# kscalelabs/kbot-joystick

Measured on AMD Instinct MI355X. Metric: env-steps/sec (whole node), K-Bot joystick 8192 envs @1/2/4/8 MI355X, higher is better.
Workload: dtype f32; 1 GPU; kbot-headless, 8192 envs/GPU, flat ground, fixed joystick command (0.5,0,0), full iteration: 100-step rollout + PPO update (batch 512/GPU, 3 passes, LSTM hidden 256, depth 2); envs_per_gpu=8192, rollout_steps=100, batch_size_per_gpu=512, num_passes=3, hidden_size=256, deterministic_update=True, parallelism=env-sharded dp1, grad all-reduce per optimizer step

## Files before the change

### kbot-joystick_amd/csrc/kbj_nn.hip

```cpp
#include <hip/hip_runtime.h>
#include <vector>
#include <cmath>
#include <cstdlib>
#include <algorithm>
#include <type_traits>
#include "kbj_ctx.h"
#include "kbj_gemm.h"
#include "kbj_nn_kernels.h"
#include "kbj_lstm_seq.h"
#include "kbj_lstm_bwd16.h"

using namespace kbj;

namespace {

constexpr int MAXD = KBJ_MAX_DEPTH;

struct NetOff {
  size_t w_in, b_in, w_ih[MAXD], w_hh[MAXD], b[MAXD], w_out, b_out;
  int nin, nout, ld_obs;
};

struct TrainBufs {
  float *obs, *X0, *G[MAXD], *Hm[MAXD], *Hout[MAXD], *Cm[MAXD], *TanhC[MAXD], *Out, *dOut, *dHa, *dHb, *dGl[MAXD];
// ... 122 lines not shown
  void* q = nullptr;
  hipError_t e = hipMalloc(&q, count * sizeof(T));
  if (e != hipSuccess) return kbj_fail(ctx, std::string("hipMalloc (nn workspace): ") + hipGetErrorString(e));
  w.allocs.push_back(q);
  *p = reinterpret_cast<T*>(q);
  return 0;
}

constexpr int g_fold_sk = 8;
#ifndef KBJ_SPLITK_WGS
#define KBJ_SPLITK_WGS 768
#endif
constexpr int g_splitk_wgs = KBJ_SPLITK_WGS;
constexpr int DETP_ROWS = 512, DETP_COLS = 4 * 512;

int lane_of(kbj_ctx* ctx, hipStream_t s) { return s == ctx->stream ? 0 : (s == ctx->stream2 ? 1 : (s == ctx->side[0] ? 2 : 3)); }
float* sk_workspace(kbj_ctx* ctx, hipStream_t s, size_t floats) {
  NnWs& w = *ws_of(ctx);
  if (!w.sched.deterministic) return nullptr;
  const int l = lane_of(ctx, s);
  if (w.skws_cap[l] < floats) {
    hipDeviceSynchronize();
    if (w.skws[l]) hipFree(w.skws[l]);
    w.skws[l] = nullptr; w.skws_cap[l] = 0;
    void* q = nullptr;
    if (hipMalloc(&q, floats * sizeof(float)) != hipSuccess) { kbj_fail(ctx, "hipMalloc (deterministic split-K workspace)"); return nullptr; }
    w.skws[l] = reinterpret_cast<float*>(q); w.skws_cap[l] = floats;
  }
  return w.skws[l];
}
float* det_partials(kbj_ctx* ctx, hipStream_t s) {
  NnWs& w = *ws_of(ctx);
  return w.sched.deterministic ? w.detp[lane_of(ctx, s)] : nullptr;
}

inline dim3 g1(size_t n, int bs = 256) { return dim3((unsigned)((n + bs - 1) / bs)); }

void linear_fwd(hipStream_t s, const float* x, int lda, const float* W, int ldw, const float* bias, float* y, int ldy, int M, int N, int K, int beta) {
  GemmArgs g{x, W, y, bias, M, N, K, lda, ldw, ldy, beta, 1, nullptr};
  gemm_launch<true, true>(s, g);
}
void linear_bwd_input(hipStream_t s, bool x3, const float* dy, int lddy, const float* W, int ldw, float* dx, int lddx, int M, int N, int K, int beta, int tile = -1) {
  GemmArgs g{dy, W, dx, nullptr, M, N, K, lddy, ldw, lddx, beta, 1, nullptr};
  g.x3 = x3;
  gemm_launch<true, false>(s, g, x3 ? -1 : tile);
}
void linear_bwd_weight(kbj_ctx* ctx, hipStream_t s, bool x3, const float* dy, int lddy, const float* x, int ldx, float* dW, int lddw, int Nout, int Nin, int R) {
  bool big = Nout >= 128 && Nin >= 128;
  int ts = big ? 128 : 64;
  int tiles = ((Nout + ts - 1) / ts) * ((Nin + ts - 1) / ts);
  int sk = std::max(2, std::min(256, g_splitk_wgs / std::max(1, tiles)));
  sk = std::max(2, std::min(sk, (R + 255) / 256));
  GemmArgs g{dy, x, dW, nullptr, Nout, Nin, R, lddy, ldx, lddw, 1, sk, nullptr};
  g.skws = sk_workspace(ctx, s, (size_t)sk * Nout * Nin);
  g.x3 = x3;
  gemm_launch<false, false>(s, g, big ? 1 : 0);
}

void linear_bwd_weight2(kbj_ctx* ctx, hipStream_t s, bool x3, const float* dy, int lddy, const float* x1, const float* x2, int ldx, float* dW1, float* dW2, int lddw, int Nout, int Nin, int R) {
  bool big = Nout >= 128 && Nin >= 128;
  int ts = big ? 128 : 64;
  if (Nin % ts != 0) {
    linear_bwd_weight(ctx, s, x3, dy, lddy, x1, ldx, dW1, lddw, Nout, Nin, R);
    linear_bwd_weight(ctx, s, x3, dy, lddy, x2, ldx, dW2, lddw, Nout, Nin, R);
    return;
  }
  int tiles = ((Nout + ts - 1) / ts) * (2 * Nin / ts);
  int sk = std::max(2, std::min(256, g_splitk_wgs / std::max(1, tiles)));
  sk = std::max(2, std::min(sk, (R + 255) / 256));
  GemmArgs g{dy, x1, dW1, nullptr, Nout, 2 * Nin, R, lddy, ldx, lddw, 1, sk, nullptr};
  g.B2 = x2; g.C2 = dW2; g.n1 = Nin;
  g.skws = sk_workspace(ctx, s, (size_t)sk * Nout * 2 * Nin);
  g.x3 = x3;
  gemm_launch<false, false>(s, g, big ? 1 : 0);
}
void colsum_acc(kbj_ctx* ctx, hipStream_t s, const float* X, int M, int N, int ld, float* out) {
  float* part = det_partials(ctx, s);
  hipLaunchKernelGGL(colsum_kernel, dim3((N + 63) / 64, DETP_ROWS), dim3(256), 0, s, X, M, N, ld, out, part);
  if (part) reduce_rows_launch(s, part, DETP_ROWS, N, out);
}

constexpr int SEQ_UW = 2;
constexpr int SEQ_FUSED_MAX_H = 256;
constexpr int SEQ_MAX_H = 512;
constexpr int SEQ_COUNTER_WORDS = 256;
constexpr int SEQ_COUNTER_TOTAL = 2 * MAXD * 4 * SEQ_COUNTER_WORDS;

template <int HC = 64, class F> bool dispatch_hidden(int H, F&& f) {
  if constexpr (HC > SEQ_MAX_H) return false;
  else return H == HC ? f(std::integral_constant<int, HC>()) : dispatch_hidden<HC + 64>(H, f);
}

int seq_fwd(kbj_ctx* ctx, hipStream_t st, int H, const SeqFwdArgs& a0) {
  SeqFwdArgs a = a0;
  a.timeout_ticks = ws_of(ctx)->seq_timeout_ticks;
  KbjKernelTimer timer(st, a.X ? (a.ldx == KBJ_LD_ACTOR ? KBJ_KIND_SEQ_FWD_OBS : KBJ_KIND_SEQ_FWD_FUSED) : KBJ_KIND_SEQ_FWD, 2.0 * a.T * a.B * 4.0 * H * (H + (a.X ? (a.kx ? a.kx : H) : 0)));
  const bool built = dispatch_hidden(H, [&](auto hc) {
    constexpr int HC = decltype(hc)::value, UW = SEQ_UW;
    int grid = (HC / (SEQ_UNITS * UW)) * ((a.B + SEQ_ROWS - 1) / SEQ_ROWS);
    if (ctx->set.seq_drop > 0 && grid > 1) { --ctx->set.seq_drop; --grid; }
    const dim3 block(256 * UW);
    if constexpr (HC <= SEQ_FUSED_MAX_H) {
      if (a.X && a.ldx == KBJ_LD_ACTOR) { hipLaunchKernelGGL((lstm_seq_fwd_kernel<HC, UW, true, KBJ_LD_ACTOR>), dim3(grid), block, 0, st, a); return true; }
      if (a.X) { hipLaunchKernelGGL((lstm_seq_fwd_kernel<HC, UW, true>), dim3(grid), block, 0, st, a); return true; }
    }
    hipLaunchKernelGGL((lstm_seq_fwd_kernel<HC, UW, false>), dim3(grid), block, 0, st, a);
    return true;
  });
  return built ? 0 : kbj_fail(ctx, "seq_fwd: the persistent LSTM kernels are built for hidden sizes 64, 128, ..., 512");
}
int seq_bwd_row_groups(int B, bool tiles16) { return tiles16 ? (B + BWD16_ROWS - 1) / BWD16_ROWS : (B + SEQ_ROWS - 1) / SEQ_ROWS; }
int seq_bwd(kbj_ctx* ctx, hipStream_t st, int H, const SeqBwdArgs& a0, bool tiles16 = false) {
  SeqBwdArgs a = a0;
  a.timeout_ticks = ws_of(ctx)->seq_timeout_ticks;
  KbjKernelTimer timer(st, tiles16 ? KBJ_KIND_SEQ_BWD16 : KBJ_KIND_SEQ_BWD, 2.0 * a.T * a.B * 4.0 * H * H);
  const bool built = dispatch_hidden(H, [&](auto hc) {
    constexpr int HC = decltype(hc)::value, UW = SEQ_UW;
    if (tiles16) {
      if constexpr (HC <= SEQ_FUSED_MAX_H) {
        int grid = (HC / BWD16_UNITS) * ((a.B + BWD16_ROWS - 1) / BWD16_ROWS);
        if (ctx->set.seq_drop_bwd > 0 && grid > 1 && HC > BWD16_UNITS) { --ctx->set.seq_drop_bwd; --grid; }
        hipLaunchKernelGGL((lstm_seq_bwd16_kernel<HC>), dim3(grid), dim3(BWD16_NTH), 0, st, a);
        return true;
      } else return false;
    }
    const dim3 grid((HC / (SEQ_UNITS * UW)) * ((a.B + SEQ_ROWS - 1) / SEQ_ROWS)), block(256 * UW);
    if constexpr (HC <= SEQ_FUSED_MAX_H) hipLaunchKernelGGL((lstm_seq_bwd_kernel<HC, UW>), grid, block, 0, st, a);
    else hipLaunchKernelGGL((lstm_seq_bwd_wide_kernel<HC, UW>), grid, block, 0, st, a);
    return true;
  });
  return built ? 0 : kbj_fail(ctx, "seq_bwd: the persistent LSTM kernels are built for hidden sizes 64, 128, ..., 512 (lstm_seq_bwd16_kernel: up to 256)");
}

template <int H> hipError_t seq_min_blocks_per_cu(int* out) {
  constexpr int threads = 256 * SEQ_UW;
  int n[4] = {0, 0, 0, 0};
  hipError_t e = hipOccupancyMaxActiveBlocksPerMultiprocessor(&n[2], lstm_seq_fwd_kernel<H, SEQ_UW, false, H>, threads, 0);
  if constexpr (H <= SEQ_FUSED_MAX_H) {
    if (e == hipSuccess) e = hipOccupancyMaxActiveBlocksPerMultiprocessor(&n[0], lstm_seq_fwd_kernel<H, SEQ_UW, true, H>, threads, 0);
    if (e == hipSuccess) e = hipOccupancyMaxActiveBlocksPerMultiprocessor(&n[1], lstm_seq_fwd_kernel<H, SEQ_UW, true, KBJ_LD_ACTOR>, threads, 0);
    if (e == hipSuccess) e = hipOccupancyMaxActiveBlocksPerMultiprocessor(&n[3], lstm_seq_bwd_kernel<H, SEQ_UW>, threads, 0);
    int n16 = 0;
    if (e == hipSuccess) e = hipOccupancyMaxActiveBlocksPerMultiprocessor(&n16, lstm_seq_bwd16_kernel<H>, BWD16_NTH, 0);
    n[3] = std::min(n[3], n16);
  } else {
    if (e == hipSuccess) e = hipOccupancyMaxActiveBlocksPerMultiprocessor(&n[3], lstm_seq_bwd_wide_kernel<H, SEQ_UW>, threads, 0);
    n[0] = n[1] = n[2];
  }
  *out = std::min(std::min(n[0], n[1]), std::min(n[2], n[3]));
  return e;
}

int lstm_step(kbj_ctx* ctx, hipStream_t st, int H, const StepArgs& a) {
  const bool obs = a.ldx == KBJ_LD_ACTOR && a.ldw == KBJ_LD_ACTOR;
  KbjKernelTimer timer(st, obs ? KBJ_KIND_LSTM_STEP_OBS : KBJ_KIND_LSTM_STEP, 2.0 * a.M * 4.0 * H * (H + (a.kx ? a.kx : H)));
  const int nug = H / (SEQ_UNITS * 2), nrg = (a.M + SEQ_ROWS - 1) / SEQ_ROWS;
  const int nch = std::max(1, std::min(nrg, 256 / nug));
  dim3 grid(nug * nch), block(512);
  const bool built = dispatch_hidden(H, [&](auto hc) {
    constexpr int HC = decltype(hc)::value;
    if constexpr (HC <= SEQ_FUSED_MAX_H) {
      if (obs) hipLaunchKernelGGL((lstm_step_kernel<HC, 2, KBJ_LD_ACTOR>), grid, block, 0, st, a);
      else hipLaunchKernelGGL((lstm_step_kernel<HC, 2>), grid, block, 0, st, a);
      return true;
    } else return false;
  });
  return built ? 0 : kbj_fail(ctx, "lstm_step: the LSTM step kernels are built for hidden_size 64, 128, 192, 256");
}

}

int kbj_nn_check_errors(kbj_ctx* ctx) {
  NnWs* w = ws_of(ctx);
  if (!w) return 0;
// ... 235 lines not shown
                       float* aux_next_d, float* qstate_t_d);

namespace {

bool net_uses_step_kernel(const NnWs& w, int n) { return w.sched.rollout_step && n == 0; }
float* h_plane(NnWs& w, float* hc, int n, int l, int n0, bool partner) {
  if (!net_uses_step_kernel(w, n)) partner = false;
  return (partner ? w.rH[n][l] : hc + (size_t)(2 * l) * w.N * w.H) + (size_t)n0 * w.H;
}

const float* fold_actor_weights(kbj_ctx* ctx, hipStream_t s, const float* params_d) {
  NnWs& w = *ws_of(ctx);
  const int H = w.H;
  if (!w.sched.rollout_step || w.net[0].ld_obs != KBJ_LD_ACTOR || !w.sched.fold_actor) return nullptr;
  const NetOff& oa = w.net[0];
  GemmArgs g{params_d + oa.w_ih[0], params_d + oa.w_in, w.Weff, nullptr, 4 * H, oa.nin, H, H, oa.nin, oa.ld_obs, 0, 1, nullptr};
  gemm_launch<true, false>(s, g);
  hipLaunchKernelGGL(matvec_kernel, dim3((4 * H + 3) / 4), dim3(256), 0, s, params_d + oa.w_ih[0], params_d + oa.b_in, params_d + oa.b[0], 4 * H, H, w.beff);
  return w.Weff;
}

void repitch_input_weights(kbj_ctx* ctx, hipStream_t s, const float* params_d, int k_lo = 0, int k_hi = 2) {
  NnWs& w = *ws_of(ctx);
  for (int k = k_lo; k < k_hi; ++k) {
    const NetOff& o = w.net[k];
    if (o.nin == o.ld_obs) continue;
    hipLaunchKernelGGL(repitch_rows_kernel, g1((size_t)w.H * o.ld_obs), dim3(256), 0, s, params_d + o.w_in, w.H, o.nin, o.ld_obs, w.WinP[k]);
  }
}

int policy_nets(kbj_ctx* ctx, hipStream_t s, const float* params_d, int net_lo, int net_hi, int n0, int cnt, const float* actor_obs_d, const float* critic_obs_d,
                kbj_carry* carry, uint32_t seed, uint32_t step_index, int argmax, float* action_d, float* logp_d, float* value_d, int parity, const float* weff) {
  NnWs& w = *ws_of(ctx);
  const kbj_config& c = ctx->cfg_h;
  const int N = w.N, H = w.H;
  const bool fused_any = w.sched.rollout_step;
  const float* obs_base[2] = {actor_obs_d, critic_obs_d};
  HeadParams hp{c.min_std, c.max_std, c.var_scale, c.lpf_alpha, w.net[0].ld_obs};
  for (int n = net_lo; n < net_hi; ++n) {
    const int k = n & 1;
    float* const hc = carry_hc(*carry, n);
    const NetOff& o = w.net[k];
    const float* obs = obs_base[k] + (size_t)n0 * o.ld_obs;
    float* obs_m = n >= 2 ? w.rObsM[k] + (size_t)n0 * o.ld_obs : nullptr;
    float* X = w.rX[n] + (size_t)n0 * H;
    float* G = w.rG[n] + (size_t)n0 * 4 * H;
    float* Out = w.rOut[n] + (size_t)n0 * 40;
    if (n >= 2) {
      hipLaunchKernelGGL(mirror_rows_kernel, g1((size_t)cnt * o.ld_obs), dim3(256), 0, s, obs, obs_m, (size_t)cnt, o.ld_obs, w.mtab[k]);
      obs = obs_m;
    }
    const bool fused = fused_any && net_uses_step_kernel(w, n);
    const bool folded = fused && weff && k == 0 && o.ld_obs == KBJ_LD_ACTOR;
    if (!folded) {
      if (o.nin != o.ld_obs) linear_fwd(s, obs, o.ld_obs, w.WinP[k], o.ld_obs, params_d + o.b_in, X, H, cnt, H, o.ld_obs, 0);
      else linear_fwd(s, obs, o.ld_obs, params_d + o.w_in, o.nin, params_d + o.b_in, X, H, cnt, H, o.nin, 0);
    }
    const float* x = X;
    for (int l = 0; l < w.D; ++l) {
      float* cc = hc + (size_t)(2 * l + 1) * N * H + (size_t)n0 * H;
      if (fused) {
        const float* h_in = h_plane(w, hc, n, l, n0, parity != 0);
        float* h_out = h_plane(w, hc, n, l, n0, parity == 0);
        StepArgs sa{x, H, 0, params_d + o.w_ih[l], H, params_d + o.w_hh[l], params_d + o.b[l], h_in, h_out, cc, cnt};
        if (l == 0 && folded) { sa.X = obs; sa.ldx = o.ld_obs; sa.kx = o.nin; sa.Wih = weff; sa.ldw = o.ld_obs; sa.bias = w.beff; }
        if (lstm_step(ctx, s, H, sa)) return -1;
        x = h_out;
        continue;
      }
      float* h = hc + (size_t)(2 * l) * N * H + (size_t)n0 * H;
      {
        GemmArgs g{x, params_d + o.w_ih[l], G, params_d + o.b[l], cnt, 4 * H, 2 * H, H, H, 4 * H, 0, 1, nullptr};
        g.A2 = h; g.B2 = params_d + o.w_hh[l]; g.k1 = H;
        g.x3 = w.sched.gemm_x3 ? 1 : 0;
        gemm_launch<true, true>(s, g, (n > 0 && w.sched.rollout_step) ? 0 : -1);
      }
      CellFwdArgs2 ca;
      ca.a[0] = CellFwdArgs{G, cc, h, cc, nullptr, nullptr, nullptr, nullptr, cnt, H};
      hipLaunchKernelGGL(lstm_cell_fwd_kernel, dim3((cnt * H + 255) / 256, 1), dim3(256), 0, s, ca);
      x = h;
    }
    if (n == 3) continue;
    if (n == 0) {
      hipLaunchKernelGGL(actor_head_fused_kernel, dim3((cnt + HEAD_ENVS * HEAD_WAVES - 1) / (HEAD_ENVS * HEAD_WAVES)), dim3(64 * HEAD_WAVES), 0, s, x, H,
                         params_d + o.w_out, params_d + o.b_out, obs, carry->lpf_d + (size_t)n0 * KBJ_NU, w.joint_bias_d, hp, seed, (uint32_t)(c.env_id_offset + n0),
                         step_index, argmax, cnt, action_d + (size_t)n0 * KBJ_NU, logp_d + n0);
      continue;
    }
    if (n == 1 && o.nout == 1) {
      hipLaunchKernelGGL(critic_value_fused_kernel, g1((size_t)cnt * 32), dim3(256), 0, s, x, H, params_d + o.w_out, params_d + o.b_out, cnt, value_d + n0);
      continue;
    }
    linear_fwd(s, x, H, params_d + o.w_out, H, params_d + o.b_out, Out, 40, cnt, o.nout, H, 0);
    hipLaunchKernelGGL(actor_head_lpf_kernel, g1((size_t)cnt * KBJ_NU), dim3(256), 0, s, Out, obs, carry->lpf_mirror_d + (size_t)n0 * KBJ_NU, w.joint_bias_d, c.lpf_alpha, cnt, w.net[0].ld_obs);
  }
  return 0;
}

void carry_reset_nets(kbj_ctx* ctx, hipStream_t s, int net_lo, int net_hi, int n0, int cnt, kbj_carry* carry, const float* done_d, int done_stride, int parity) {
  NnWs& w = *ws_of(ctx);
  float* lpf[4] = {carry->lpf_d, nullptr, carry->lpf_mirror_d, nullptr};
  const bool partner = parity != 0 && w.sched.rollout_step;
  for (int k = net_lo; k < net_hi; ++k) {
    float* const hc = carry_hc(*carry, k);
    CarryPlanes cp;
    cp.n = 2 * w.D;
    for (int l = 0; l < w.D; ++l) {
      cp.p[2 * l] = h_plane(w, hc, k, l, n0, partner);
      cp.p[2 * l + 1] = hc + (size_t)(2 * l + 1) * w.N * w.H + (size_t)n0 * w.H;
    }
    hipLaunchKernelGGL(carry_reset_kernel, dim3((cnt + 3) / 4), dim3(256), 0, s, cp, cnt, w.H, lpf[k] ? lpf[k] + (size_t)n0 * KBJ_NU : nullptr, done_d + (size_t)n0 * done_stride, done_stride);
  }
}

int carry_h_home(kbj_ctx* ctx, hipStream_t s, int net_lo, int net_hi, kbj_carry* carry) {
  NnWs& w = *ws_of(ctx);
  for (int k = net_lo; k < net_hi; ++k)
    for (int l = 0; l < w.D && net_uses_step_kernel(w, k); ++l)
      KBJ_HIP(ctx, hipMemcpyAsync(carry_hc(*carry, k) + (size_t)(2 * l) * w.N * w.H, w.rH[k][l], (size_t)w.N * w.H * sizeof(float), hipMemcpyDeviceToDevice, s));
  return 0;
}

void pad_params(kbj_ctx* ctx, hipStream_t s, const float* user, float* internal) {
  NnWs& w = *ws_of(ctx);
  hipLaunchKernelGGL(pad_params_kernel, g1(w.nparams), dim3(256), 0, s, w.pad_desc, w.npad, const_cast<float*>(user), internal, w.nparams, 0);
}
void unpad_params(kbj_ctx* ctx, hipStream_t s, const float* internal, float* user) {
  NnWs& w = *ws_of(ctx);
  hipLaunchKernelGGL(pad_params_kernel, g1(w.nparams), dim3(256), 0, s, w.pad_desc, w.npad, user, const_cast<float*>(internal), w.nparams, 1);
}
void repitch_hc(kbj_ctx* ctx, hipStream_t s, const float* src, float* dst, int ws, int wd) {
  NnWs& w = *ws_of(ctx);
  const size_t rows = (size_t)2 * w.D * w.N;
  hipLaunchKernelGGL(repitch_pad_kernel, g1(rows * wd), dim3(256), 0, s, src, dst, rows, ws, wd);
}
kbj_carry pad_carry(kbj_ctx* ctx, hipStream_t s, const kbj_carry& c) {
  NnWs& w = *ws_of(ctx);
  kbj_carry p = c;
  for (int k = 0; k < 4; ++k)
    if (carry_hc(c, k) && w.phc[k]) { repitch_hc(ctx, s, carry_hc(c, k), w.phc[k], w.Hu, w.H); carry_hc(p, k) = w.phc[k]; }
  return p;
}
void unpad_carry(kbj_ctx* ctx, hipStream_t s, const kbj_carry& c) {
  NnWs& w = *ws_of(ctx);
  for (int k = 0; k < 4; ++k)
    if (carry_hc(c, k) && w.phc[k]) repitch_hc(ctx, s, w.phc[k], carry_hc(c, k), w.H, w.Hu);
}
kbj_traj pad_traj_carry0(kbj_ctx* ctx, hipStream_t s, const kbj_traj& tr) {
  NnWs& w = *ws_of(ctx);
  kbj_traj p = tr;
  for (int k = 0; k < 4; ++k)
    if (traj_carry0(tr, k) && w.pc0[k]) { repitch_hc(ctx, s, traj_carry0(tr, k), w.pc0[k], w.Hu, w.H); traj_carry0(p, k) = w.pc0[k]; }
  return p;
}

int critic_tail(kbj_ctx* ctx, hipStream_t s, const float* params_d, const float* critic_obs_d, const float* critic_hc_d, int hc_width, float* value_d) {
  NnWs& w = *ws_of(ctx);
  if (hc_width == w.H) KBJ_HIP(ctx, hipMemcpyAsync(w.tail_hc, critic_hc_d, (size_t)2 * w.D * w.N * w.H * sizeof(float), hipMemcpyDeviceToDevice, s));
  else repitch_hc(ctx, s, critic_hc_d, w.tail_hc, hc_width, w.H);
  kbj_carry sc = {};
  sc.critic_hc_d = w.tail_hc;
  return policy_nets(ctx, s, params_d, 1, 2, 0, w.N, nullptr, critic_obs_d, &sc, 0, 0, 0, nullptr, nullptr, value_d, 0, nullptr);
}

int policy_step_body(kbj_ctx* ctx, const float* params_d, const float* actor_obs_d, const float* critic_obs_d, kbj_carry* carry, uint32_t seed,
                     uint32_t step_index, int argmax, float* action_d, float* logp_d, float* value_d) {
  NnWs& w = *ws_of(ctx);
  kbj_nn_drop_prefetch(ctx);
  KbjTimed timed(ctx, true);
// ... 632 lines not shown
```

### kbot-joystick_amd/csrc/kbj_nn_kernels.h

```cpp
#pragma once
#include <hip/hip_runtime.h>
#include <stdint.h>
#include "kbj_model.h"

namespace kbj {

constexpr float kLog2Pi = 1.8378770664093453f;

__device__ __forceinline__ float sigmoidf_(float x) { return __builtin_amdgcn_rcpf(1.0f + __expf(-x)); }
__device__ __forceinline__ float tanhf_(float x) { float xc = fminf(fmaxf(x, -15.0f), 15.0f); return 1.0f - 2.0f * __builtin_amdgcn_rcpf(1.0f + __expf(2.0f * xc)); }
__device__ __forceinline__ float softplusf_(float x) { return x > 20.0f ? x : log1pf(expf(x)); }

struct CellFwdArgs {
  float* G; const float* c_prev; float* h_out; float* c_out; float* hm_next; float* cm_next; float* tanhc; const float* keep;
  int M, H;
};
struct CellFwdArgs2 { CellFwdArgs a[2]; };
__global__ void lstm_cell_fwd_kernel(CellFwdArgs2 args) {
  const CellFwdArgs& a = args.a[blockIdx.y];
  int idx = blockIdx.x * blockDim.x + threadIdx.x;
  if (idx >= a.M * a.H) return;
  int m = idx / a.H, u = idx - m * a.H;
  float* g = a.G + (size_t)m * 4 * a.H;
  float i = sigmoidf_(g[u]), f = sigmoidf_(g[a.H + u]), gg = tanhf_(g[2 * a.H + u]), o = sigmoidf_(g[3 * a.H + u]);
  float c = f * a.c_prev[idx] + i * gg;
  float tc = tanhf_(c), h = o * tc;
  g[u] = i; g[a.H + u] = f; g[2 * a.H + u] = gg; g[3 * a.H + u] = o;
  a.h_out[idx] = h;
  a.c_out[idx] = c;
  if (a.hm_next) { float k = a.keep[m]; a.hm_next[idx] = h * k; a.cm_next[idx] = c * k; a.tanhc[idx] = tc; }
}

__device__ __forceinline__ uint32_t nn_rotl32(uint32_t x, int r) { return (x << r) | (x >> (32 - r)); }
__device__ __forceinline__ void nn_threefry(uint32_t k0, uint32_t k1, uint32_t c0, uint32_t c1, uint32_t& o0, uint32_t& o1) {
  const int rot[8] = {13, 15, 26, 6, 17, 29, 16, 24};
  uint32_t ks[3] = {k0, k1, k0 ^ k1 ^ 0x1BD11BDAu};
  uint32_t x0 = c0 + ks[0], x1 = c1 + ks[1];
#pragma unroll
  for (int g = 0; g < 5; ++g) {
#pragma unroll
    for (int r = 0; r < 4; ++r) { x0 += x1; x1 = nn_rotl32(x1, rot[(g & 1) * 4 + r]); x1 ^= x0; }
    x0 += ks[(g + 1) % 3]; x1 += ks[(g + 2) % 3] + (uint32_t)(g + 1);
  }
  o0 = x0; o1 = x1;
}

struct HeadParams { float min_std, max_std, var_scale, alpha; int ld_obs; };
constexpr int HEAD_ENVS = 16;
constexpr int HEAD_WAVES = 4;
typedef float head_f32x4 __attribute__((ext_vector_type(4)));
__global__ __launch_bounds__(64 * HEAD_WAVES) void actor_head_fused_kernel(const float* __restrict__ hin , int H, const float* __restrict__ Wout ,
                                                                          const float* __restrict__ bout, const float* __restrict__ obs ,
                                                                          float* __restrict__ lpf, const float* __restrict__ joint_bias, HeadParams hp, uint32_t seed,
                                                                          uint32_t env_off, uint32_t step, int argmax, int N, float* __restrict__ action,
                                                                          float* __restrict__ logp) {
  __shared__ float outs[HEAD_WAVES][HEAD_ENVS][49];
  __shared__ float lps[HEAD_WAVES][HEAD_ENVS][KBJ_NU + 1];
  const int lane = threadIdx.x & 63, wv = threadIdx.x >> 6, g = lane >> 4, c = lane & 15;
  const int n0 = (blockIdx.x * HEAD_WAVES + wv) * HEAD_ENVS;
  if (n0 < N) {
    const float* arow = hin + (size_t)min(n0 + c, N - 1) * H + 4 * g;
    const float* brow[3] = {Wout + (size_t)c * H + 4 * g, Wout + (size_t)(16 + c) * H + 4 * g, Wout + (size_t)min(32 + c, 2 * KBJ_NU - 1) * H + 4 * g};
    head_f32x4 acc[3] = {{0, 0, 0, 0}, {0, 0, 0, 0}, {0, 0, 0, 0}};
    for (int k = 0; k < H; k += 16) {
      const head_f32x4 a = *reinterpret_cast<const head_f32x4*>(arow + k);
#pragma unroll
      for (int t = 0; t < 3; ++t) {
        const head_f32x4 b = *reinterpret_cast<const head_f32x4*>(brow[t] + k);
#pragma unroll
        for (int q = 0; q < 4; ++q) acc[t] = __builtin_amdgcn_mfma_f32_16x16x4f32(a[q], b[q], acc[t], 0, 0, 0);
      }
    }
#pragma unroll
    for (int t = 0; t < 3; ++t)
#pragma unroll
      for (int r = 0; r < 4; ++r) outs[wv][4 * g + r][16 * t + c] = acc[t][r];
  }
  __syncthreads();
  if (n0 < N) {
    for (int item = lane; item < HEAD_ENVS * KBJ_NU; item += 64) {
      const int e = item / KBJ_NU, j = item - e * KBJ_NU, n = n0 + e;
      float lp = 0;
      if (n < N) {
        const float om = outs[wv][e][j] + bout[j], os = outs[wv][e][KBJ_NU + j] + bout[KBJ_NU + j];
        float mean = om + joint_bias[j] + (j >= 10 ? obs[(size_t)n * hp.ld_obs + KBJ_OBS_CMD + 6 + (j - 10)] : 0.0f);
        float sd = fminf((softplusf_(os) + hp.min_std) * hp.var_scale, hp.max_std);
        float y0 = lpf[n * KBJ_NU + j];
        float y = y0 + hp.alpha * (mean - y0);
        lpf[n * KBJ_NU + j] = y;
        float a = y;
        if (!argmax) {
          uint32_t b0, b1;
          nn_threefry(seed ^ ((uint32_t)KBJ_RNG_ACTION * 0x9E3779B9u), env_off + (uint32_t)n, step, (uint32_t)j, b0, b1);
          float u1 = (float)((b0 >> 8) + 1u) * (1.0f / 16777216.0f), u2 = (float)(b1 >> 8) * (1.0f / 16777216.0f);
          a = y + sd * (sqrtf(-2.0f * logf(u1)) * cosf(6.283185307179586f * u2));
        }
        action[n * KBJ_NU + j] = a;
        float z = (a - y) / sd;
        lp = -0.5f * z * z - logf(sd) - 0.5f * kLog2Pi;
      }
      lps[wv][e][j] = lp;
    }
  }
  __syncthreads();
  if (n0 < N && lane < HEAD_ENVS && n0 + lane < N) {
    float lp = 0;
#pragma unroll
    for (int j = 0; j < KBJ_NU; ++j) lp += lps[wv][lane][j];
    logp[n0 + lane] = lp;
  }
}

__global__ __launch_bounds__(256) void critic_value_fused_kernel(const float* __restrict__ hin , int H, const float* __restrict__ wout ,
                                                                 const float* __restrict__ bout, int N, float* __restrict__ value) {
  const int tid = blockIdx.x * blockDim.x + threadIdx.x, n = tid >> 5, j = tid & 31;
  float acc = 0;
  if (n < N)
    for (int c = j; c < H / 4; c += 32) {
      const float4 h = *reinterpret_cast<const float4*>(hin + (size_t)n * H + 4 * c), w = *reinterpret_cast<const float4*>(wout + 4 * c);
      acc = fmaf(h.x, w.x, acc); acc = fmaf(h.y, w.y, acc); acc = fmaf(h.z, w.z, acc); acc = fmaf(h.w, w.w, acc);
    }
  for (int o = 16; o > 0; o >>= 1) acc += __shfl_xor(acc, o);
  if (n < N && j == 0) value[n] = acc + bout[0];
}

__global__ void critic_value_kernel(const float* __restrict__ out, int ld, int N, float* __restrict__ value) {
  int n = blockIdx.x * blockDim.x + threadIdx.x;
  if (n < N) value[n] = out[(size_t)n * ld];
}

struct CarryPlanes { float* p[2 * KBJ_MAX_DEPTH]; int n; };
__global__ void carry_reset_kernel(CarryPlanes hc, int cnt, int H, float* __restrict__ lpf, const float* __restrict__ done, int stride) {
  const int row = blockIdx.x * (blockDim.x >> 6) + (threadIdx.x >> 6), lane = threadIdx.x & 63;
  if (row >= cnt || done[(size_t)row * stride] == 0.0f) return;
  for (int p = 0; p < hc.n; ++p)
    for (int k = lane; k < H; k += 64) hc.p[p][(size_t)row * H + k] = 0.0f;
  if (lpf && lane < KBJ_NU) lpf[(size_t)row * KBJ_NU + lane] = 0.0f;
}

__global__ void gather_rows_kernel(const float* __restrict__ src, const int* __restrict__ idx, int T, int N, int B, int w, int ld_src, int ld_dst, float* __restrict__ dst) {
  size_t i = (size_t)blockIdx.x * blockDim.x + threadIdx.x;
  size_t total = (size_t)T * B * w;
  if (i >= total) return;
  int k = i % w;
  size_t r = i / w;
  int b = r % B, t = r / B;
  dst[r * ld_dst + k] = src[((size_t)t * N + idx[b]) * ld_src + k];
}
__global__ void gather_rows4_kernel(const float4* __restrict__ src, const int* __restrict__ idx, int T, int N, int B, int w4, int ld_src4, int ld_dst4, float4* __restrict__ dst) {
  size_t i = (size_t)blockIdx.x * blockDim.x + threadIdx.x;
  size_t total = (size_t)T * B * w4;
  if (i >= total) return;
  int k = i % w4;
  size_t r = i / w4;
  int b = r % B, t = r / B;
  dst[r * ld_dst4 + k] = src[((size_t)t * N + idx[b]) * ld_src4 + k];
}
__global__ void gather_keep_kernel(const float* __restrict__ aux, const int* __restrict__ idx, int T, int N, int B, float* __restrict__ keep) {
  int i = blockIdx.x * blockDim.x + threadIdx.x;
  if (i >= T * B) return;
  int b = i % B, t = i / B;
  keep[i] = aux[((size_t)t * N + idx[b]) * KBJ_AUX_SIZE + KBJ_AUX_DONE] != 0 ? 0.0f : 1.0f;
}

struct GatherSmallArgs {
  const float *action, *logp, *value, *adv, *target, *aux;
  float *action_o, *logp_o, *value_o, *adv_o, *target_o, *keep_o;
};
__global__ void gather_small_kernel(GatherSmallArgs a, const int* __restrict__ idx, int T, int N, int B, int c0, int c1) {
  const int W = c1 - c0;
  size_t i = (size_t)blockIdx.x * blockDim.x + threadIdx.x;
  if (i >= (size_t)T * B * W) return;
  size_t r = i / W;
  int c = c0 + (int)(i - r * W), b = (int)(r % B);
  size_t src = (r / B) * N + idx[b];
  if (c < KBJ_NU) a.action_o[r * KBJ_NU + c] = a.action[src * KBJ_NU + c];
  else if (c == KBJ_NU) { if (a.logp) a.logp_o[r] = a.logp[src]; }
  else if (c == KBJ_NU + 1) { if (a.value) a.value_o[r] = a.value[src]; }
  else if (c == KBJ_NU + 2) { if (a.adv) a.adv_o[r] = a.adv[src]; }
  else if (c == KBJ_NU + 3) { if (a.target) a.target_o[r] = a.target[src]; }
  else a.keep_o[r] = a.aux[src * KBJ_AUX_SIZE + KBJ_AUX_DONE] != 0 ? 0.0f : 1.0f;
}
struct GatherCarryArgs { const float* src[8 * KBJ_MAX_DEPTH + 2]; float* dst[8 * KBJ_MAX_DEPTH + 2]; int nplanes, nlpf; };
__global__ void gather_carry_kernel(GatherCarryArgs a, const int* __restrict__ idx, int B, int H) {
  int p = blockIdx.y;
  int w = p < a.nplanes ? H : KBJ_NU;
  int i = blockIdx.x * blockDim.x + threadIdx.x;
  if (i >= B * w) return;
  int b = i / w, k = i - b * w;
  a.dst[p][i] = a.src[p][(size_t)idx[b] * w + k];
}

__global__ void actor_head_pre_kernel(const float* __restrict__ out, const float* __restrict__ obs, const float* __restrict__ joint_bias, HeadParams hp,
// ... 455 lines not shown
```

Measured before the change: 2.332 million env-steps/s.

## Split actor head output tiles across waves and batch K loads with templated hidden size

The fused actor head kernel used to have each wave compute all three 16-column output tiles for its own 16 envs, looping over K. It now gives each block 16 envs and three waves, one per output tile. The hidden size becomes a template parameter so the K loop fully unrolls, and all A/B loads for a chunk are issued before the MFMAs, with sched barriers between them. This is meant to raise parallelism and memory-level overlap in a latency-bound kernel, at the cost of more blocks, redundant loads of the hidden rows across waves, and higher register pressure.

```diff
diff --git a/kbot-joystick_amd/csrc/kbj_nn.hip b/kbot-joystick_amd/csrc/kbj_nn.hip
--- a/kbot-joystick_amd/csrc/kbj_nn.hip
+++ b/kbot-joystick_amd/csrc/kbj_nn.hip
@@ -228,14 +228,8 @@
 
 constexpr int SEQ_UW = 2;
 constexpr int SEQ_FUSED_MAX_H = 256;
-constexpr int SEQ_MAX_H = 512;
 constexpr int SEQ_COUNTER_WORDS = 256;
 constexpr int SEQ_COUNTER_TOTAL = 2 * MAXD * 4 * SEQ_COUNTER_WORDS;
-
-template <int HC = 64, class F> bool dispatch_hidden(int H, F&& f) {
-  if constexpr (HC > SEQ_MAX_H) return false;
-  else return H == HC ? f(std::integral_constant<int, HC>()) : dispatch_hidden<HC + 64>(H, f);
-}
 
 int seq_fwd(kbj_ctx* ctx, hipStream_t st, int H, const SeqFwdArgs& a0) {
   SeqFwdArgs a = a0;
@@ -637,9 +631,9 @@
     }
     if (n == 3) continue;
     if (n == 0) {
-      hipLaunchKernelGGL(actor_head_fused_kernel, dim3((cnt + HEAD_ENVS * HEAD_WAVES - 1) / (HEAD_ENVS * HEAD_WAVES)), dim3(64 * HEAD_WAVES), 0, s, x, H,
-                         params_d + o.w_out, params_d + o.b_out, obs, carry->lpf_d + (size_t)n0 * KBJ_NU, w.joint_bias_d, hp, seed, (uint32_t)(c.env_id_offset + n0),
-                         step_index, argmax, cnt, action_d + (size_t)n0 * KBJ_NU, logp_d + n0);
+      const HeadArgs ha{x, params_d + o.w_out, params_d + o.b_out, obs, carry->lpf_d + (size_t)n0 * KBJ_NU, w.joint_bias_d, hp, seed, (uint32_t)(c.env_id_offset + n0),
+                        step_index, argmax, cnt, action_d + (size_t)n0 * KBJ_NU, logp_d + n0};
+      if (!actor_head_launch(s, H, ha)) return kbj_fail(ctx, "policy_nets: the actor head is built for hidden sizes 64, 128, ..., 512");
       continue;
     }
     if (n == 1 && o.nout == 1) {
diff --git a/kbot-joystick_amd/csrc/kbj_nn_kernels.h b/kbot-joystick_amd/csrc/kbj_nn_kernels.h
--- a/kbot-joystick_amd/csrc/kbj_nn_kernels.h
+++ b/kbot-joystick_amd/csrc/kbj_nn_kernels.h
@@ -1,6 +1,7 @@
 #pragma once
 #include <hip/hip_runtime.h>
 #include <stdint.h>
+#include <type_traits>
 #include "kbj_model.h"
 
 namespace kbj {
@@ -46,69 +47,92 @@
 }
 
 struct HeadParams { float min_std, max_std, var_scale, alpha; int ld_obs; };
+
+constexpr int SEQ_MAX_H = 512;
+template <int HC = 64, class F> bool dispatch_hidden(int H, F&& f) {
+  if constexpr (HC > SEQ_MAX_H) return false;
+  else return H == HC ? f(std::integral_constant<int, HC>()) : dispatch_hidden<HC + 64>(H, f);
+}
+
+struct HeadArgs {
+  const float* hin ; const float* Wout ; const float* bout; const float* obs ; float* lpf; const float* joint_bias;
+  HeadParams hp; uint32_t seed, env_off, step; int argmax, N; float* action; float* logp;
+};
+__device__ __forceinline__ float head_joint(const HeadArgs& p, int n, int j, float om_raw, float os_raw) {
+  const HeadParams& hp = p.hp;
+  const float om = om_raw + p.bout[j], os = os_raw + p.bout[KBJ_NU + j];
+  float mean = om + p.joint_bias[j] + (j >= 10 ? p.obs[(size_t)n * hp.ld_obs + KBJ_OBS_CMD + 6 + (j - 10)] : 0.0f);
+  float sd = fminf((softplusf_(os) + hp.min_std) * hp.var_scale, hp.max_std);
+  float y0 = p.lpf[n * KBJ_NU + j];
+  float y = y0 + hp.alpha * (mean - y0);
+  p.lpf[n * KBJ_NU + j] = y;
+  float a = y;
+  if (!p.argmax) {
+    uint32_t b0, b1;
+    nn_threefry(p.seed ^ ((uint32_t)KBJ_RNG_ACTION * 0x9E3779B9u), p.env_off + (uint32_t)n, p.step, (uint32_t)j, b0, b1);
+    float u1 = (float)((b0 >> 8) + 1u) * (1.0f / 16777216.0f), u2 = (float)(b1 >> 8) * (1.0f / 16777216.0f);
+    a = y + sd * (sqrtf(-2.0f * logf(u1)) * cosf(6.283185307179586f * u2));
+  }
+  p.action[n * KBJ_NU + j] = a;
+  float z = (a - y) / sd;
+  return -0.5f * z * z - logf(sd) - 0.5f * kLog2Pi;
+}
+
 constexpr int HEAD_ENVS = 16;
-constexpr int HEAD_WAVES = 4;
+constexpr int HEAD_TILES = 3;
+constexpr int HEAD_CHUNK = 16;
 typedef float head_f32x4 __attribute__((ext_vector_type(4)));
-__global__ __launch_bounds__(64 * HEAD_WAVES) void actor_head_fused_kernel(const float* __restrict__ hin , int H, const float* __restrict__ Wout ,
-                                                                          const float* __restrict__ bout, const float* __restrict__ obs ,
-                                                                          float* __restrict__ lpf, const float* __restrict__ joint_bias, HeadParams hp, uint32_t seed,
-                                                                          uint32_t env_off, uint32_t step, int argmax, int N, float* __restrict__ action,
-                                                                          float* __restrict__ logp) {
-  __shared__ float outs[HEAD_WAVES][HEAD_ENVS][49];
-  __shared__ float lps[HEAD_WAVES][HEAD_ENVS][KBJ_NU + 1];
-  const int lane = threadIdx.x & 63, wv = threadIdx.x >> 6, g = lane >> 4, c = lane & 15;
-  const int n0 = (blockIdx.x * HEAD_WAVES + wv) * HEAD_ENVS;
-  if (n0 < N) {
-    const float* arow = hin + (size_t)min(n0 + c, N - 1) * H + 4 * g;
-    const float* brow[3] = {Wout + (size_t)c * H + 4 * g, Wout + (size_t)(16 + c) * H + 4 * g, Wout + (size_t)min(32 + c, 2 * KBJ_NU - 1) * H + 4 * g};
-    head_f32x4 acc[3] = {{0, 0, 0, 0}, {0, 0, 0, 0}, {0, 0, 0, 0}};
-    for (int k = 0; k < H; k += 16) {
-      const head_f32x4 a = *reinterpret_cast<const head_f32x4*>(arow + k);
-#pragma unroll
-      for (int t = 0; t < 3; ++t) {
-        const head_f32x4 b = *reinterpret_cast<const head_f32x4*>(brow[t] + k);
-#pragma unroll
-        for (int q = 0; q < 4; ++q) acc[t] = __builtin_amdgcn_mfma_f32_16x16x4f32(a[q], b[q], acc[t], 0, 0, 0);
-      }
-    }
-#pragma unroll
-    for (int t = 0; t < 3; ++t)
-#pragma unroll
-      for (int r = 0; r < 4; ++r) outs[wv][4 * g + r][16 * t + c] = acc[t][r];
-  }
-  __syncthreads();
-  if (n0 < N) {
-    for (int item = lane; item < HEAD_ENVS * KBJ_NU; item += 64) {
-      const int e = item / KBJ_NU, j = item - e * KBJ_NU, n = n0 + e;
-      float lp = 0;
-      if (n < N) {
-        const float om = outs[wv][e][j] + bout[j], os = outs[wv][e][KBJ_NU + j] + bout[KBJ_NU + j];
-        float mean = om + joint_bias[j] + (j >= 10 ? obs[(size_t)n * hp.ld_obs + KBJ_OBS_CMD + 6 + (j - 10)] : 0.0f);
-        float sd = fminf((softplusf_(os) + hp.min_std) * hp.var_scale, hp.max_std);
-        float y0 = lpf[n * KBJ_NU + j];
-        float y = y0 + hp.alpha * (mean - y0);
-        lpf[n * KBJ_NU + j] = y;
-        float a = y;
-        if (!argmax) {
-          uint32_t b0, b1;
-          nn_threefry(seed ^ ((uint32_t)KBJ_RNG_ACTION * 0x9E3779B9u), env_off + (uint32_t)n, step, (uint32_t)j, b0, b1);
-          float u1 = (float)((b0 >> 8) + 1u) * (1.0f / 16777216.0f), u2 = (float)(b1 >> 8) * (1.0f / 16777216.0f);
-          a = y + sd * (sqrtf(-2.0f * logf(u1)) * cosf(6.283185307179586f * u2));
+template <int H>
+__global__ __launch_bounds__(64 * HEAD_TILES) void actor_head_rows_kernel(HeadArgs p) {
+  static_assert(H % 16 == 0, "k blocks of 16");
+  __shared__ float outs[HEAD_ENVS][49];
+  __shared__ float lps[HEAD_ENVS][KBJ_NU + 1];
+  const int lane = threadIdx.x & 63, t = threadIdx.x >> 6, g = lane >> 4, c = lane & 15;
+  const int n0 = blockIdx.x * HEAD_ENVS, N = p.N;
+  {
+    const float* arow = p.hin + (size_t)min(n0 + c, N - 1) * H + 4 * g;
+    const float* brow = p.Wout + (size_t)min(16 * t + c, 2 * KBJ_NU - 1) * H + 4 * g;
+    head_f32x4 acc = {0, 0, 0, 0};
+    constexpr int KB = H / 16;
+#pragma unroll
+    for (int k0 = 0; k0 < KB; k0 += HEAD_CHUNK) {
+      head_f32x4 a[HEAD_CHUNK], b[HEAD_CHUNK];
+#pragma unroll
+      for (int i = 0; i < HEAD_CHUNK; ++i)
+        if (k0 + i < KB) {
+          a[i] = *reinterpret_cast<const head_f32x4*>(arow + 16 * (k0 + i));
+          b[i] = *reinterpret_cast<const head_f32x4*>(brow + 16 * (k0 + i));
         }
-        action[n * KBJ_NU + j] = a;
-        float z = (a - y) / sd;
-        lp = -0.5f * z * z - logf(sd) - 0.5f * kLog2Pi;
-      }
-      lps[wv][e][j] = lp;
-    }
-  }
-  __syncthreads();
-  if (n0 < N && lane < HEAD_ENVS && n0 + lane < N) {
+      __builtin_amdgcn_sched_barrier(0);
+#pragma unroll
+      for (int i = 0; i < HEAD_CHUNK; ++i)
+        if (k0 + i < KB) {
+#pragma unroll
+          for (int q = 0; q < 4; ++q) acc = __builtin_amdgcn_mfma_f32_16x16x4f32(a[i][q], b[i][q], acc, 0, 0, 0);
+        }
+      __builtin_amdgcn_sched_barrier(0);
+    }
+#pragma unroll
+    for (int r = 0; r < 4; ++r) outs[4 * g + r][16 * t + c] = acc[r];
+  }
+  __syncthreads();
+  for (int item = threadIdx.x; item < HEAD_ENVS * KBJ_NU; item += 64 * HEAD_TILES) {
+    const int e = item / KBJ_NU, j = item - e * KBJ_NU, n = n0 + e;
+    lps[e][j] = n < N ? head_joint(p, n, j, outs[e][j], outs[e][KBJ_NU + j]) : 0.0f;
+  }
+  __syncthreads();
+  if (threadIdx.x < HEAD_ENVS && n0 + threadIdx.x < N) {
     float lp = 0;
 #pragma unroll
-    for (int j = 0; j < KBJ_NU; ++j) lp += lps[wv][lane][j];
-    logp[n0 + lane] = lp;
-  }
+    for (int j = 0; j < KBJ_NU; ++j) lp += lps[threadIdx.x][j];
+    p.logp[n0 + threadIdx.x] = lp;
+  }
+}
+inline bool actor_head_launch(hipStream_t s, int H, const HeadArgs& a) {
+  return dispatch_hidden(H, [&](auto hc) {
+    hipLaunchKernelGGL((actor_head_rows_kernel<decltype(hc)::value>), dim3((a.N + HEAD_ENVS - 1) / HEAD_ENVS), dim3(64 * HEAD_TILES), 0, s, a);
+    return true;
+  });
 }
 
 __global__ __launch_bounds__(256) void critic_value_fused_kernel(const float* __restrict__ hin , int H, const float* __restrict__ wout ,
```

Result: no change. 2.338 million env-steps/s, median of 6 (+0.3%).
